# secondmind-labs/trieste

Measured on NVIDIA H100. Metric: acquisition candidate-points/sec (EI on GPR N=4096 fp64), higher is better.
Workload: dtype f64

## Files before the change

trieste_b200/csrc/digit_gemm.cuh:

```cuda
#pragma once
#include "common.cuh"
#include "kernel_fn.cuh"

namespace tb {
namespace oz {

constexpr int KST = 64;
constexpr uint32_t LBO = 128;
constexpr uint32_t SBO = (KST / 16) * 128;
constexpr int ATILE = 128 * KST;

__host__ __device__ inline int64_t a_stage_offset(int I) {
  return (int64_t)I * (I + 1);
}

template <int POS, int SRC>
__device__ __forceinline__ uint32_t put_byte(uint32_t acc, uint32_t w) {
  constexpr uint32_t sel = (POS == 0 ? (4u + SRC) : 0u) | ((POS == 1 ? (4u + SRC) : 1u) << 4) | ((POS == 2 ? (4u + SRC) : 2u) << 8) |
                           ((POS == 3 ? (4u + SRC) : 3u) << 12);
  return __byte_perm(acc, w, sel);
}

}

namespace dg {

using oz::ATILE;
using oz::KST;
using oz::LBO;
using oz::SBO;

constexpr int STAGES = 3;
constexpr int CONSUMER_WARPS = 8;
constexpr int THREADS = CONSUMER_WARPS * 32 + 128;
constexpr int PRODUCER_REGS = 40, CONSUMER_REGS = 232;
enum { EPI_SUMSQ = 0, EPI_STORE = 1 };

template <int S> __host__ __device__ constexpr int chunk_cols() { return S >= 6 ? 32 : 64; }
template <int S> __host__ __device__ constexpr int stage_bytes() { return S * (ATILE + chunk_cols<S>() * KST); }
template <int S> __host__ __device__ constexpr size_t smem_bytes() {
  return (size_t)STAGES * stage_bytes<S>() + 256 + (size_t)CONSUMER_WARPS * chunk_cols<S>() * sizeof(double);
}

__device__ __forceinline__ uint64_t smem_desc(uint32_t saddr) {
  return (uint64_t)((saddr >> 4) & 0x3FFF) | ((uint64_t)((LBO >> 4) & 0x3FFF) << 16) | ((uint64_t)((SBO >> 4) & 0x3FFF) << 32);
}

__device__ __forceinline__ void wgmma_fence() { asm volatile("wgmma.fence.sync.aligned;" ::: "memory"); }
__device__ __forceinline__ void wgmma_commit() { asm volatile("wgmma.commit_group.sync.aligned;" ::: "memory"); }
template <int N>
__device__ __forceinline__ void wgmma_wait() { asm volatile("wgmma.wait_group.sync.aligned %0;" ::"n"(N) : "memory"); }

template <int R>
// ... 28 lines not shown
}
#undef TB_R4

template <int S, int NR>
__device__ __forceinline__ void fence_acc(uint32_t (&acc)[S][NR]) {
#pragma unroll
  for (int l = 0; l < S; ++l)
#pragma unroll
    for (int i = 0; i < NR; ++i) asm volatile("" : "+r"(acc[l][i])::"memory");
}

__device__ __forceinline__ double int_to_double(uint32_t t) {
  return __hiloint2double(0x43300000, (int)(t ^ 0x80000000u)) - 4503601774854144.0;
}

template <int S, int EPI, int NTB>
__global__ void __launch_bounds__(THREADS, 1)
digit_gemm_kernel(const int8_t* __restrict__ AS, const int8_t* __restrict__ BS, const double* __restrict__ rowscale,
                  const double* __restrict__ rowsum, int NB, int nst, int G, int tiles, int64_t McPad, double out_scale,
                  double half_var, int a_planes, int b_planes, int full_rows, double* __restrict__ partial,
                  double* __restrict__ Aplain, int64_t lda) {
  constexpr int CN = chunk_cols<S>(), NCH = NTB / CN, BCH = CN * KST, BTILE = NTB * KST, STAGE = stage_bytes<S>(), NR = CN / 2;
  static_assert(NTB % CN == 0, "a candidate tile is a whole number of column chunks");
  extern __shared__ __align__(1024) unsigned char smem[];
  uint64_t* full = reinterpret_cast<uint64_t*>(smem + (size_t)STAGES * STAGE);
  uint64_t* empty = full + STAGES;
  double (*colbuf)[CN] = reinterpret_cast<double (*)[CN]>(smem + (size_t)STAGES * STAGE + 256);

  const int warp = threadIdx.x >> 5, lane = threadIdx.x & 31;
  const int nitems = tiles * NCH * G;
  if (threadIdx.x == 0) {
    for (int s = 0; s < STAGES; ++s) {
      mbar_init(&full[s], 1);
      mbar_init(&empty[s], CONSUMER_WARPS);
    }
    fence_barrier_init();
  }
  for (int i = threadIdx.x; i < CONSUMER_WARPS * CN; i += blockDim.x) colbuf[i / CN][i % CN] = 0.0;
  __syncthreads();

  if (warp >= CONSUMER_WARPS) {
    setmaxnreg_dec<PRODUCER_REGS>();
    if (warp == CONSUMER_WARPS && lane == 0) {
      int st = 0;
      uint32_t ph = 0;
      for (int item = blockIdx.x; item < nitems; item += gridDim.x) {
        const int g = item % G, tc = item / G, tile = tc / NCH, c = tc % NCH;
        const int8_t* bTile = BS + (int64_t)tile * nst * ((int64_t)b_planes * BTILE) + (int64_t)c * BCH;
        for (int i = 0;; ++i) {
          const int I = serpentine_rowblock(i, g, G);
          if (I >= NB) break;
          const int nk = full_rows ? nst : min(2 * (I + 1), nst);
          const int8_t* aRow = AS + (full_rows ? (int64_t)I * nst : oz::a_stage_offset(I)) * ((int64_t)a_planes * ATILE);
          for (int kc = 0; kc < nk; ++kc) {
            mbar_wait(&empty[st], ph ^ 1);
            unsigned char* dst = smem + (size_t)st * STAGE;
            mbar_expect_tx(&full[st], STAGE);
            bulk_g2s(dst, aRow + (int64_t)kc * ((int64_t)a_planes * ATILE), S * ATILE, &full[st]);
            const int8_t* b = bTile + (int64_t)kc * ((int64_t)b_planes * BTILE);
#pragma unroll
            for (int p = 0; p < S; ++p) bulk_g2s(dst + S * ATILE + p * BCH, b + (int64_t)p * BTILE, BCH, &full[st]);
            if (++st == STAGES) { st = 0; ph ^= 1; }
          }
        }
      }
    }
    return;
  }

  setmaxnreg_inc<CONSUMER_REGS>();
  const int wg = warp >> 2, wq = warp & 3;
  const uint32_t a_lane = (uint32_t)((wg * 8 + wq * 2 + ((lane >> 3) & 1)) * (int)SBO + (lane >> 4) * (int)LBO + (lane & 7) * 16);
  uint32_t acc[S][NR];
  int st = 0;
  uint32_t ph = 0;
  for (int item = blockIdx.x; item < nitems; item += gridDim.x) {
    const int g = item % G, tc = item / G, tile = tc / NCH, c = tc % NCH;
    for (int i = 0;; ++i) {
      const int I = serpentine_rowblock(i, g, G);
      if (I >= NB) break;
      const int nk = full_rows ? nst : min(2 * (I + 1), nst);
#pragma unroll
      for (int l = 0; l < S; ++l)
#pragma unroll
        for (int j = 0; j < NR; ++j) acc[l][j] = 0u;
      fence_acc(acc);
      int held = -1;
      for (int kc = 0; kc < nk; ++kc) {
        mbar_wait(&full[st], ph);
        const uint32_t base = smem_u32(smem + (size_t)st * STAGE);
        const uint64_t b0 = smem_desc(base + (uint32_t)(S * ATILE));
#pragma unroll
        for (int p = 1; p <= S; ++p) {
          uint32_t a[KST / 32][4];
#pragma unroll
          for (int kk = 0; kk < KST / 32; ++kk) ldmatrix_x4(a[kk], base + a_lane + (uint32_t)((p - 1) * ATILE + kk * 2 * (int)LBO));
          wgmma_wait<1>();
          if (p == 2 && held >= 0) {
            __syncwarp();
            if (lane == 0) mbar_arrive(&empty[held]);
          }
          wgmma_fence();
#pragma unroll
          for (int q = 1; q <= S + 1 - p; ++q)
#pragma unroll
            for (int kk = 0; kk < KST / 32; ++kk) wgmma_s8(acc[p + q - 2], a[kk], b0 + (uint64_t)(((q - 1) * BCH + kk * 2 * (int)LBO) >> 4));
          wgmma_commit();
        }
        held = st;
        if (++st == STAGES) { st = 0; ph ^= 1; }
      }
      wgmma_wait<0>();
      fence_acc(acc);
      __syncwarp();
      if (lane == 0) mbar_arrive(&empty[held]);
      const int64_t r0 = (int64_t)I * 128 + wg * 64 + wq * 16 + (lane >> 2), r1 = r0 + 8;
      const double rs0 = rowscale[r0] * out_scale * 0x1p-16, rs1 = rowscale[r1] * out_scale * 0x1p-16;
      const double rc0 = rowsum ? rowsum[r0] * half_var : 0.0, rc1 = rowsum ? rowsum[r1] * half_var : 0.0;
#pragma unroll
      for (int j = 0; j < CN / 8; ++j) {
        double a[4];
#pragma unroll
        for (int e = 0; e < 4; ++e) {
          double v = int_to_double(acc[S - 1][4 * j + e]);
#pragma unroll
          for (int l = S - 2; l >= 0; --l) v = fma(v, 0x1p-8, int_to_double(acc[l][4 * j + e]));
          a[e] = e < 2 ? fma(v, rs0, rc0) : fma(v, rs1, rc1);
        }
        const int col = 8 * j + 2 * (lane & 3);
        if (EPI == EPI_STORE) {
          double* dst = Aplain + ((int64_t)tile * NTB + (int64_t)c * CN + col) * lda;
          dst[r0] = a[0];
          dst[lda + r0] = a[1];
          dst[r1] = a[2];
          dst[lda + r1] = a[3];
        } else {
          double s0 = fma(a[0], a[0], a[2] * a[2]), s1 = fma(a[1], a[1], a[3] * a[3]);
#pragma unroll
          for (int o = 4; o < 32; o <<= 1) {
            s0 += __shfl_xor_sync(0xffffffffu, s0, o);
            s1 += __shfl_xor_sync(0xffffffffu, s1, o);
          }
          if (lane < 4) {
            colbuf[warp][col] += s0;
            colbuf[warp][col + 1] += s1;
          }
        }
      }
    }
    if (EPI == EPI_SUMSQ) {
      asm volatile("bar.sync 1, %0;" ::"n"(CONSUMER_WARPS * 32) : "memory");
      if (threadIdx.x < CN) {
        double s = 0.0;
#pragma unroll
        for (int w = 0; w < CONSUMER_WARPS; ++w) {
          s += colbuf[w][threadIdx.x];
          colbuf[w][threadIdx.x] = 0.0;
        }
        partial[(int64_t)g * McPad + (int64_t)tile * NTB + (int64_t)c * CN + threadIdx.x] = s;
      }
      asm volatile("bar.sync 1, %0;" ::"n"(CONSUMER_WARPS * 32) : "memory");
    }
  }
}

inline int sm_count(int* n) {
  int dev = 0;
  TB_CUDA(cudaGetDevice(&dev));
  TB_CUDA(cudaDeviceGetAttribute(n, cudaDevAttrMultiProcessorCount, dev));
  return 0;
}

template <int S, int EPI, int NTB>
inline int set_smem() {
  TB_CUDA(cudaFuncSetAttribute(digit_gemm_kernel<S, EPI, NTB>, cudaFuncAttributeMaxDynamicSharedMemorySize, (int)smem_bytes<S>()));
  return 0;
}

template <int S, int EPI, int NTB>
inline int launch(cudaStream_t st, const int8_t* AS, const int8_t* BS, const double* rowscale, const double* rowsum, int NB, int nst,
                  int G, int tiles, int64_t McPad, double out_scale, double half_var, int a_planes, int b_planes, int full_rows,
                  double* partial, double* Aplain, int64_t lda) {
  int sms = 0;
  TB_TRY(sm_count(&sms));
  const int64_t items = (int64_t)tiles * (NTB / chunk_cols<S>()) * G;
  const int grid = (int)std::min<int64_t>(sms, items);
  if (grid <= 0) return 0;
  digit_gemm_kernel<S, EPI, NTB><<<grid, THREADS, smem_bytes<S>(), st>>>(AS, BS, rowscale, rowsum, NB, nst, G, tiles, McPad, out_scale,
                                                                         half_var, a_planes, b_planes, full_rows, partial, Aplain, lda);
  TB_LAUNCHED();
  TB_CUDA(cudaGetLastError());
  return 0;
}

}
}
```

trieste_b200/csrc/gp_handle.cuh:

```cuda
#pragma once
#include "common.cuh"
#include "../../include/trieste_b200.h"
#include <cublas_v2.h>
#include <cusolverDn.h>
#include <vector>
#include <algorithm>
#include <cmath>
#include <cstdlib>
#include <type_traits>
#include <utility>

namespace tb {

struct DevBuf {
  void* p = nullptr;
  size_t cap = 0;
  DevBuf() = default;
  DevBuf(const DevBuf&) = delete;
  DevBuf& operator=(const DevBuf&) = delete;
  DevBuf(DevBuf&& o) noexcept : p(o.p), cap(o.cap) {
    o.p = nullptr;
    o.cap = 0;
  }
  DevBuf& operator=(DevBuf&& o) noexcept {
// ... 155 lines not shown
  tb::DevBuf sKs, sPartial, sMean, sVals, sVar, sXc, sBlkBest, sBlkIdx, sRun;
  tb::DevBuf sA, sV, sGrad, sMisc;
  tb::DevBuf dXspare, dyspare, dLspare, dLinvSpare;
  tb::DevBuf dMes;
  int mesS = 0;
  tb::DevBuf dPen;
  int penP = 0, penKind = 0, penD = 0;
  std::vector<double> gibP;
  int gibM = 0, gibMp = 0, gibD = 0;
  double gibW = 0.0;
  uint64_t cache_gen = 0;
  uint64_t gib_gen = tb::STALE;
  tb::DevBuf dGibPs, dGibLinv, dGibWhat;
  tb::DevBuf sGib;
  tb::DevBuf sScrUb, sScrX, sScrIdx, sScrBlk;
  tb::DevBuf dPreRows, dPreCentre;
  uint64_t pre_gen = tb::STALE;
  bool pre_tc = false;
  int pre_nsl = 0, pre_npos_sl = 0;
  double pre_scale = 1.0, pre_x2max = 0.0, pre_rel = 0.0, pre_lin = 0.0, pre_lin_max = 0.0, pre_abs = 0.0;

  bool profile = false;
  double prof_ms = 0.0, prof_flops = 0.0;
  int64_t prof_launches = 0;
  std::vector<std::pair<cudaEvent_t, cudaEvent_t>> prof_events;
  std::vector<double> prof_event_flops;
};
```

trieste_b200/csrc/int8_engines.cu:

```cuda
#include "gp_handle.cuh"
#include "ozaki5.cuh"
#include "int8_engines.h"

namespace tb {

int int8_init() {
  TB_TRY((dg::set_smem<6, dg::EPI_SUMSQ, oz::Geo<6>::NT>()));
  TB_TRY((dg::set_smem<6, dg::EPI_STORE, oz::Geo<6>::NT>()));
  TB_TRY((dg::set_smem<5, dg::EPI_SUMSQ, oz::Geo<5>::NT>()));
  TB_TRY((dg::set_smem<5, dg::EPI_STORE, oz::Geo<5>::NT>()));
  TB_TRY((dg::set_smem<4, dg::EPI_SUMSQ, oz::Geo<4>::NT>()));
  TB_TRY((dg::set_smem<4, dg::EPI_STORE, oz::Geo<4>::NT>()));
  TB_TRY((dg::set_smem<3, dg::EPI_SUMSQ, oz::Geo<3>::NT>()));
  return 0;
}

static int nst_of(const tb_gp* gp) { return (int)((gp->N + oz::KST - 1) / oz::KST); }

static int stored_planes(const tb_gp* gp, bool single_pass) { return single_pass ? gp->digits.linv.planes : oz::S21; }
int int8_tile_width(const tb_gp* gp, bool single_pass) {
  return stored_planes(gp, single_pass) == 5 ? oz::Geo<5>::NT : oz::Geo<6>::NT;
}
size_t int8_tile_bytes(const tb_gp* gp, bool single_pass) {
  return (size_t)nst_of(gp) * stored_planes(gp, single_pass) * int8_tile_width(gp, single_pass) * oz::KST;
}


static int row_stats(tb_gp* gp, DigitOperand& o, const double* A, int full, bool tight) {
// ... 160 lines not shown
  const double* il = gp->dInvLs.as<double>();
  const int N = (int)gp->N, nst = nst_of(gp), D = gp->D;
  const double var = gp->variance, mc0 = gp->mean_const;
  const double inv_b = std::ldexp(1.0, 48 - bscale_exp(var));
  cudaStream_t st = gp->stream;
  with_kind_dp(gp->kernel, gp->DP, [&](auto K, auto P) {
    oz::kstar_digits_kernel<decltype(K)::value, decltype(P)::value><<<tiles, 512, 0, st>>>(Xs, al, Xc_dev, il, N, nst, D, mc, var, inv_b,
                                                                                            mc0, BS, mean);
  });
  TB_LAUNCHED();
  TB_CUDA(cudaGetLastError());
  return 0;
}

template <int S>
static int kstar_single_pass(tb_gp* gp, const double* Xc_dev, int64_t mc, int tiles, int8_t* BS, double* mean, const KSplit* split) {
  const double* Xs = gp->dXs.as<double>();
  const double* al = gp->dAlpha.as<double>();
  const double* il = gp->dInvLs.as<double>();
  const int N = (int)gp->N, nst = nst_of(gp), D = gp->D;
  const double var = gp->variance, mc0 = gp->mean_const;
  const double inv_b = oz::two_pow_8S<S>() * oz::FILL / (0.5 * var);
  const double dig_c = fm::MAGIC + oz5::dig_koff<S>() - centre_int(S);
  const double* X2 = gp->digits.X2.as<double>();
  cudaStream_t st = gp->stream;
  constexpr int TH = oz5::KGEN_WARPS * 32;
  const unsigned ctas = kstar_ctas<S>(tiles);
  const KSplit ks = split ? *split : int8_kstar_split(gp, true, tiles);
  const int ksplit = ks.ksplit, kc_per = ks.kc_per;
  const int64_t mstride = (int64_t)tiles * oz::Geo<S>::NT;
  double* mean_dst = mean;
  if (ksplit > 1) {
    TB_TRY(gp->sMeanPart.reserve(sizeof(double) * (size_t)ksplit * mstride));
    mean_dst = gp->sMeanPart.as<double>();
  }
  with_kind_dp(gp->kernel, gp->DP, [&](auto K, auto P) {
    oz5::kstar_digits_kernel<decltype(K)::value, decltype(P)::value, S><<<dim3(ctas, ksplit), TH, 0, st>>>(
        Xs, X2, al, Xc_dev, il, N, nst, D, mc, var, inv_b, dig_c, mc0, fm::Consts(), tiles, kc_per, BS, mean_dst);
  });
  TB_LAUNCHED();
  if (ksplit > 1) {
    oz5::mean_reduce_kernel<<<(unsigned)((mstride + 255) / 256), 256, 0, st>>>(mean_dst, ksplit, mstride, mc0, mean);
    TB_LAUNCHED();
  }
  TB_CUDA(cudaGetLastError());
  return 0;
}

int int8_kstar(tb_gp* gp, bool single_pass, const double* Xc_dev, int64_t mc, int tiles, int8_t* BS, double* mean,
               const KSplit* split) {
  if (!single_pass) return kstar_21(gp, Xc_dev, mc, tiles, BS, mean);
  return gp->digits.linv.planes == 5 ? kstar_single_pass<5>(gp, Xc_dev, mc, tiles, BS, mean, split)
                                     : kstar_single_pass<4>(gp, Xc_dev, mc, tiles, BS, mean, split);
}


template <int EPI>
static int digit_gemm(tb_gp* gp, const DigitOperand& left, int full_rows, int S, double out_scale, double h, const int8_t* BS,
                      int tiles, int G, int64_t McPad, double* partial, double* out, int64_t lda) {
  auto launch = [&](auto SV) {
    constexpr int s = decltype(SV)::value;
    return dg::launch<s, EPI, oz::Geo<s>::NT>(gp->stream, left.digits.as<int8_t>(), BS, left.scale.as<double>(), left.sum.as<double>(),
                                              gp->NB, nst_of(gp), G, tiles, McPad, out_scale, h, left.planes, left.planes, full_rows,
                                              partial, out, lda);
  };
  switch (S) {
    case 6: return launch(std::integral_constant<int, 6>{});
    case 5: return launch(std::integral_constant<int, 5>{});
    case 4: return launch(std::integral_constant<int, 4>{});
  }
  if constexpr (EPI == dg::EPI_SUMSQ) return launch(std::integral_constant<int, 3>{});
  return fail("digit GEMM: no store kernel computes with " + std::to_string(S) + " digits", ERR_RUNTIME);
}

int int8_variance(tb_gp* gp, bool single_pass, const int8_t* BS, int tiles, int G, int64_t McPad, double* partial) {
  const DigitState& d = gp->digits;
  const double var = gp->variance;
  if (single_pass)
    return digit_gemm<dg::EPI_SUMSQ>(gp, d.linv, 0, d.mode, 0.5 * var / oz::FILL, h_eff(var, d.linv.planes), BS, tiles, G, McPad,
                                     partial, nullptr, 0);
  return digit_gemm<dg::EPI_SUMSQ>(gp, d.linv21, 0, gp->dtype == TB_F32 ? 4 : 6, std::ldexp(1.0, bscale_exp(var)), 0.0, BS, tiles, G,
                                   McPad, partial, nullptr, 0);
}

int int8_store(tb_gp* gp, bool single_pass, bool kinv, const int8_t* BS, int tiles, int G, int64_t McPad, double* out, int64_t lda) {
  const DigitState& d = gp->digits;
  const double var = gp->variance;
  if (single_pass) {
    const DigitOperand& left = kinv ? d.kinv : d.linv;
    return digit_gemm<dg::EPI_STORE>(gp, left, kinv, left.planes, 0.5 * var / oz::FILL, h_eff(var, left.planes), BS, tiles, G, McPad,
                                     nullptr, out, lda);
  }
  return digit_gemm<dg::EPI_STORE>(gp, kinv ? d.kinv21 : d.linv21, kinv, gp->dtype == TB_F32 ? 4 : 6, std::ldexp(1.0, bscale_exp(var)),
                                   0.0, BS, tiles, G, McPad, nullptr, out, lda);
}

}
// ... 1 lines not shown
```

trieste_b200/csrc/int8_engines.h:

```cpp
#pragma once
#include <cuda_runtime.h>
#include <cstddef>
#include <cstdint>
struct tb_gp;
namespace tb {
int int8_init();
int int8_select(tb_gp* gp, bool need_v, bool* single_pass);
int int8_tile_width(const tb_gp* gp, bool single_pass);
size_t int8_tile_bytes(const tb_gp* gp, bool single_pass);
struct KSplit {
  int ksplit = 1, kc_per = 0;
};
KSplit int8_kstar_split(const tb_gp* gp, bool single_pass, int tiles);
int int8_kstar(tb_gp* gp, bool single_pass, const double* Xc_dev, int64_t mc, int tiles, int8_t* BS, double* mean,
               const KSplit* split = nullptr);
int int8_variance(tb_gp* gp, bool single_pass, const int8_t* BS, int tiles, int G, int64_t McPad, double* partial);
int int8_store(tb_gp* gp, bool single_pass, bool kinv, const int8_t* BS, int tiles, int G, int64_t McPad, double* out, int64_t lda);
void int8_info(const tb_gp* gp, int* products, double* estimate);
void int8_pin_full(tb_gp* gp, bool full);
}
```

trieste_b200/csrc/ozaki5.cuh:

```cuda
#pragma once
#include "ozaki.cuh"

namespace tb {
namespace oz5 {

using oz::FILL;
using oz::Geo;
using oz::KST;
using oz::LBO;
using oz::SBO;
using oz::two_pow_8S;

template <int S> __host__ __device__ constexpr double dig_koff() { return S == 5 ? 551911719040.0 : S == 4 ? 2155905152.0 : 8421504.0; }

__global__ void row_norms_kernel(const double* __restrict__ Xs, int64_t rows_have, int DP, int64_t rows, double* __restrict__ X2) {
  const int64_t k = (int64_t)blockIdx.x * blockDim.x + threadIdx.x;
  if (k >= rows) return;
  double s = 0.0;
  if (k < rows_have)
    for (int d = 0; d < DP; ++d) s = fma(Xs[k * DP + d], Xs[k * DP + d], s);
  X2[k] = s;
}

constexpr int KGEN_WARPS = 8;
template <int KIND, int DP, int S>
__global__ void __launch_bounds__(KGEN_WARPS * 32, DP <= 12 ? 4 : 3)
kstar_digits_kernel(const double* __restrict__ Xs, const double* __restrict__ X2, const double* __restrict__ alpha,
                    const double* __restrict__ Xc, const double* __restrict__ inv_ls, int N, int nst, int D, int64_t M, double variance,
                    double inv_bscale_2p, double dig_c, double mean_const, const __grid_constant__ fm::Consts fc, int ntiles,
                    int kc_per, int8_t* __restrict__ BS, double* __restrict__ mean_out) {
  constexpr int NT = Geo<S>::NT, BTILE = NT * KST, TH = KGEN_WARPS * 32, WPT = NT / 8;
  constexpr bool EXPAND = KIND != TB_MATERN12;
  const int lane = threadIdx.x & 31;
  const int64_t wg = (int64_t)blockIdx.x * KGEN_WARPS + (threadIdx.x >> 5);
  const int64_t tile_id = wg / WPT;
  const int w = (int)(wg % WPT);
  const int cl = lane & 7, ch = lane >> 3;
  const int t_local = w * 8 + cl;
  const int64_t t = tile_id * NT + t_local;
  const bool valid = t < M && tile_id < ntiles;
  double xc[DP];
// ... 20 lines not shown
      if (e < CH) asm volatile("cp.async.ca.shared.global [%0], [%1], 16;" ::"r"(smem_u32(&xs_s[buf][2 * e + 2 * blk])), "l"(src + 2 * e) : "memory");
    }
    if (threadIdx.x < KST / 2) {
      const int e = threadIdx.x;
      asm volatile("cp.async.ca.shared.global [%0], [%1], 16;" ::"r"(smem_u32(&al_s[buf][2 * e + 2 * (e / 8)])), "l"(alpha + (int64_t)kc * KST + 2 * e)
                   : "memory");
    } else if (EXPAND && threadIdx.x < KST) {
      const int e = threadIdx.x - KST / 2;
      asm volatile("cp.async.ca.shared.global [%0], [%1], 16;" ::"r"(smem_u32(&x2_s[buf][2 * e + 2 * (e / 8)])), "l"(X2 + (int64_t)kc * KST + 2 * e)
                   : "memory");
    }
    asm volatile("cp.async.commit_group;" ::: "memory");
  };
  const int kc0 = (int)blockIdx.y * kc_per, kc1 = min(nst, kc0 + kc_per);
  stage_load(kc0, 0);
  double macc = 0.0;
  for (int kc = kc0; kc < kc1; ++kc) {
    const int buf = (kc - kc0) & 1;
    if (kc + 1 < kc1) {
      stage_load(kc + 1, buf ^ 1);
      asm volatile("cp.async.wait_group 1;" ::: "memory");
    } else {
      asm volatile("cp.async.wait_group 0;" ::: "memory");
    }
    __syncthreads();
    uint32_t pk[S][4];
#pragma unroll
    for (int p = 0; p < S; ++p) pk[p][0] = pk[p][1] = pk[p][2] = pk[p][3] = 0u;
#pragma unroll
    for (int j = 0; j < 16; ++j) {
      const int kl = ch * 16 + j, kv = kl + 2 * ch;
// ... 7 lines not shown
          dot = fma(xc[d], v.x, dot);
          dot = fma(xc[d + 1], v.y, dot);
        }
        r2 = fma(-2.0, dot, xc2 + x2_s[buf][kv]);
      } else {
        r2 = 0.0;
#pragma unroll
        for (int d = 0; d < DP; d += 2) {
          const double2 v = *reinterpret_cast<const double2*>(xr + d);
          double d0 = xc[d] - v.x, d1 = xc[d + 1] - v.y;
          r2 = fma(d0, d0, r2);
          r2 = fma(d1, d1, r2);
        }
      }
      const double kval = kernel_from_r2_fast<KIND>(r2, variance, exp_tab, fc);
      macc = fma(kval, al_s[buf][kv], macc);
      const double tb = fma(kval, inv_bscale_2p, dig_c);
      const uint32_t wl = (uint32_t)__double2loint(tb) ^ 0x80808080u, wh = (uint32_t)__double2hiint(tb) ^ 0x80u;
      oz::scatter_rt<S>(pk, j, wl, wh);
    }
    if (tile_id < ntiles) {
#pragma unroll
      for (int p = 0; p < S; ++p)
        *reinterpret_cast<uint4*>(tile + (int64_t)kc * (S * BTILE) + p * BTILE) = make_uint4(pk[p][0], pk[p][1], pk[p][2], pk[p][3]);
    }
    __syncthreads();
  }
  macc += __shfl_xor_sync(0xffffffffu, macc, 8);
  macc += __shfl_xor_sync(0xffffffffu, macc, 16);
  if (ch == 0 && tile_id < ntiles)
    mean_out[(int64_t)blockIdx.y * ntiles * NT + tile_id * NT + t_local] = gridDim.y == 1 ? macc + mean_const : macc;
}

__global__ void mean_reduce_kernel(const double* __restrict__ part, int ksplit, int64_t stride, double mean_const,
                                   double* __restrict__ mean_out) {
  const int64_t t = (int64_t)blockIdx.x * blockDim.x + threadIdx.x;
  if (t >= stride) return;
  double s = 0.0;
  for (int i = 0; i < ksplit; ++i) s += part[(int64_t)i * stride + t];
  mean_out[t] = s + mean_const;
}

}
}
```

trieste_b200/csrc/tb_api.cu:

```cuda
#include "gp_handle.cuh"
#include "kernels_extra.cuh"
#include "prescreen.cuh"
#include "batch_ei.cuh"
#include "int8_engines.h"
#include <chrono>
#include "factor.cuh"
#include "lbfgs.cuh"

using namespace tb;
namespace tb {
int kernels_init();
}

namespace tb {

__global__ void scale_inputs_kernel(const double* __restrict__ X, const double* __restrict__ inv_ls,
                                    int64_t N, int D, int DP, int64_t rows, double* __restrict__ Xs) {
  int64_t i = (int64_t)blockIdx.x * blockDim.x + threadIdx.x;
  if (i >= rows * DP) return;
  int64_t k = i / DP;
  int d = (int)(i % DP);
  Xs[i] = (k < N && d < D) ? X[k * D + d] * inv_ls[d] : 0.0;
}

// ... 1065 lines not shown
  *eng = single_pass ? Engine::OZ15 : Engine::OZ21;
  return 0;
}

static int eng_tile_width(const tb_gp* gp, Engine e) { return e == Engine::F64 ? BT : int8_tile_width(gp, e == Engine::OZ15); }
static size_t eng_tile_bytes(const tb_gp* gp, Engine e) {
  return e == Engine::F64 ? (size_t)gp->nkc * PANEL * sizeof(double) : int8_tile_bytes(gp, e == Engine::OZ15);
}

static int eng_groups(const tb_gp* gp, Engine e, int tiles) {
  const int fill = (2 * NUM_SMS + tiles - 1) / tiles;
  if (e == Engine::F64) return tiles >= NUM_SMS ? 1 : std::max(1, std::min(fill, gp->NB));
  return std::max(std::max(1, (gp->NB + 3) / 4), std::min(gp->NB, fill));
}

static int eng_kstar(tb_gp* gp, Engine e, const double* xc, int64_t mc, int tiles, const KSplit* split = nullptr) {
  double* mean = gp->sMean.as<double>();
  if (e == Engine::F64) return launch_kstar(gp, xc, mc, tiles, gp->sKs.as<double>(), mean);
  return int8_kstar(gp, e == Engine::OZ15, xc, mc, tiles, gp->sKs.as<int8_t>(), mean, split);
}

static int eng_variance(tb_gp* gp, Engine e, int tiles, int G, int64_t McPad, bool packed_a) {
  cudaStream_t st = gp->stream;
  double* partial = gp->sPartial.as<double>();
  if (e != Engine::F64) return int8_variance(gp, e == Engine::OZ15, gp->sKs.as<int8_t>(), tiles, G, McPad, partial);
  if (packed_a)
    trigemm_kernel<false, EPI_SUMSQ_PACKED><<<dim3(tiles, G), TG_THREADS, TG_SMEM, st>>>(
        gp->dLinvP.as<double>(), gp->sKs.as<double>(), gp->NB, gp->nkc, G, McPad, partial, gp->sA.as<double>(), nullptr, 0);
  else
    trigemm_kernel<false, EPI_SUMSQ><<<dim3(tiles, G), TG_THREADS, TG_SMEM, st>>>(
        gp->dLinvP.as<double>(), gp->sKs.as<double>(), gp->NB, gp->nkc, G, McPad, partial, nullptr, nullptr, 0);
  TB_LAUNCHED();
  TB_CUDA(cudaGetLastError());
  return 0;
}

static int eng_store_a(tb_gp* gp, Engine e, int tiles, int64_t McPad, double* out) {
  const int64_t lda = (int64_t)gp->NB * BM;
  const int G = eng_groups(gp, e, tiles);
  if (e != Engine::F64) return int8_store(gp, e == Engine::OZ15, false, gp->sKs.as<int8_t>(), tiles, G, McPad, out, lda);
// ... 68 lines not shown
  return 0;
}

struct EvalOut {
  double *vals = nullptr, *mean = nullptr, *var = nullptr, *grad = nullptr;
};

static int eval_chunk(tb_gp* gp, const EvalRequest& rq, Engine e, const double* xc, int64_t n, int64_t c0, int G, const EvalOut& o,
                      const int64_t* idx_map = nullptr, const KSplit* split = nullptr) {
  cudaStream_t st = gp->stream;
  const int nt = eng_tile_width(gp, e);
  const int tiles = (int)((n + nt - 1) / nt);
  const int64_t McPad = (int64_t)tiles * nt;
  const double* partial = gp->sPartial.as<double>();
  const double* mean = gp->sMean.as<double>();
  TB_TRY(eng_kstar(gp, e, xc, n, tiles, split));
  TB_TRY(profiled_gemm(gp, (double)McPad * (double)gp->N * (double)gp->N,
                       [&] { return eng_variance(gp, e, tiles, G, McPad, o.grad != nullptr); }));
  if (o.grad) {
    TB_TRY(launch_partials(gp, st, rq.acq, rq.param, partial, G, McPad, mean, xc, n));
    TB_TRY(eng_store_v(gp, e, tiles, McPad));
    TB_TRY(launch_grad(gp, xc, n, o.grad));
  }
  TB_TRY(launch_tail(gp, st, rq, partial, G, McPad, mean, n, c0, o.vals, o.mean, o.var, xc, o.grad, idx_map));
  return rq.want_argmax ? argmax_fold(gp, n) : 0;
}

static int argmax_screened(tb_gp* gp, const EvalRequest& rq, Engine e, int64_t chunk_cap, int G, bool* done) {
  *done = false;
  cudaStream_t st = gp->stream;
  const int D = gp->D, nt = eng_tile_width(gp, e);
  const int64_t M = rq.M;
  const int64_t cap = std::max<int64_t>(1, M / 4);
// ... 1517 lines not shown
```

Before: 275.9 million.

## Add split-K digit GEMM and wide k-star generation for small candidate batches

When there are too few candidate tiles to fill the SMs (the screened-argmax path with an index map), the int8 digit GEMM splits each row block's K range across CTAs. Partial integer accumulators are combined with atomics into a global buffer and a separate epilogue kernel turns them into variance partial sums. The k-star generation also switches to a wide grid split over K stages, writing kernel values to global memory so that a replay kernel computes the mean. This raises parallelism for small batches at the cost of extra memsets, atomics, global traffic and kernel launches.

```diff
diff --git a/trieste_b200/csrc/digit_gemm.cuh b/trieste_b200/csrc/digit_gemm.cuh
--- a/trieste_b200/csrc/digit_gemm.cuh
+++ b/trieste_b200/csrc/digit_gemm.cuh
@@ -34,9 +34,10 @@
 constexpr int CONSUMER_WARPS = 8;
 constexpr int THREADS = CONSUMER_WARPS * 32 + 128;
 constexpr int PRODUCER_REGS = 40, CONSUMER_REGS = 232;
-enum { EPI_SUMSQ = 0, EPI_STORE = 1 };
-
-template <int S> __host__ __device__ constexpr int chunk_cols() { return S >= 6 ? 32 : 64; }
+enum { EPI_SUMSQ = 0, EPI_STORE = 1, EPI_SPLIT = 2 };
+
+__host__ __device__ constexpr int chunk_cols_of(int S) { return S >= 6 ? 32 : 64; }
+template <int S> __host__ __device__ constexpr int chunk_cols() { return chunk_cols_of(S); }
 template <int S> __host__ __device__ constexpr int stage_bytes() { return S * (ATILE + chunk_cols<S>() * KST); }
 template <int S> __host__ __device__ constexpr size_t smem_bytes() {
   return (size_t)STAGES * stage_bytes<S>() + 256 + (size_t)CONSUMER_WARPS * chunk_cols<S>() * sizeof(double);
@@ -95,12 +96,99 @@
   return __hiloint2double(0x43300000, (int)(t ^ 0x80000000u)) - 4503601774854144.0;
 }
 
+__host__ __device__ inline int rowblock_stages(int I, int nst, int full_rows) { return full_rows ? nst : min(2 * (I + 1), nst); }
+
+__host__ __device__ inline int split_units(int NB, int nst, int full_rows, int kper) {
+  int u = 0;
+  for (int I = 0; I < NB; ++I) u += (rowblock_stages(I, nst, full_rows) + kper - 1) / kper;
+  return u;
+}
+
+template <int EPI>
+__device__ __forceinline__ bool item_range(int g, int i, int G, int NB, int nst, int full_rows, int kper, int& I, int& k0, int& k1) {
+  if constexpr (EPI == EPI_SPLIT) {
+    if (i > 0) return false;
+    for (I = 0; I < NB; ++I) {
+      const int nk = rowblock_stages(I, nst, full_rows), p = (nk + kper - 1) / kper;
+      if (g < p) {
+        k0 = g * kper;
+        k1 = min(nk, k0 + kper);
+        return true;
+      }
+      g -= p;
+    }
+    return false;
+  } else {
+    I = serpentine_rowblock(i, g, G);
+    k0 = 0;
+    k1 = rowblock_stages(I, nst, full_rows);
+    return I < NB;
+  }
+}
+
+template <int S, int EPI, int NTB>
+__device__ __forceinline__ void rowblock_epilogue(const uint32_t (&acc)[S][chunk_cols<S>() / 2], int I, int tile, int c, int warp, int lane,
+                                                  const double* __restrict__ rowscale, const double* __restrict__ rowsum,
+                                                  double out_scale, double half_var, double (*colbuf)[chunk_cols<S>()],
+                                                  double* __restrict__ Aplain, int64_t lda) {
+  constexpr int CN = chunk_cols<S>();
+  const int wg = warp >> 2, wq = warp & 3;
+  const int64_t r0 = (int64_t)I * 128 + wg * 64 + wq * 16 + (lane >> 2), r1 = r0 + 8;
+  const double rs0 = rowscale[r0] * out_scale * 0x1p-16, rs1 = rowscale[r1] * out_scale * 0x1p-16;
+  const double rc0 = rowsum ? rowsum[r0] * half_var : 0.0, rc1 = rowsum ? rowsum[r1] * half_var : 0.0;
+#pragma unroll
+  for (int j = 0; j < CN / 8; ++j) {
+    double a[4];
+#pragma unroll
+    for (int e = 0; e < 4; ++e) {
+      double v = int_to_double(acc[S - 1][4 * j + e]);
+#pragma unroll
+      for (int l = S - 2; l >= 0; --l) v = fma(v, 0x1p-8, int_to_double(acc[l][4 * j + e]));
+      a[e] = e < 2 ? fma(v, rs0, rc0) : fma(v, rs1, rc1);
+    }
+    const int col = 8 * j + 2 * (lane & 3);
+    if constexpr (EPI == EPI_STORE) {
+      double* dst = Aplain + ((int64_t)tile * NTB + (int64_t)c * CN + col) * lda;
+      dst[r0] = a[0];
+      dst[lda + r0] = a[1];
+      dst[r1] = a[2];
+      dst[lda + r1] = a[3];
+    } else {
+      double s0 = fma(a[0], a[0], a[2] * a[2]), s1 = fma(a[1], a[1], a[3] * a[3]);
+#pragma unroll
+      for (int o = 4; o < 32; o <<= 1) {
+        s0 += __shfl_xor_sync(0xffffffffu, s0, o);
+        s1 += __shfl_xor_sync(0xffffffffu, s1, o);
+      }
+      if (lane < 4) {
+        colbuf[warp][col] += s0;
+        colbuf[warp][col + 1] += s1;
+      }
+    }
+  }
+}
+
+template <int CN>
+__device__ __forceinline__ void colbuf_flush(double (*colbuf)[CN], double* __restrict__ dst) {
+  asm volatile("bar.sync 1, %0;" ::"n"(CONSUMER_WARPS * 32) : "memory");
+  if (threadIdx.x < CN) {
+    double s = 0.0;
+#pragma unroll
+    for (int w = 0; w < CONSUMER_WARPS; ++w) {
+      s += colbuf[w][threadIdx.x];
+      colbuf[w][threadIdx.x] = 0.0;
+    }
+    dst[threadIdx.x] = s;
+  }
+  asm volatile("bar.sync 1, %0;" ::"n"(CONSUMER_WARPS * 32) : "memory");
+}
+
 template <int S, int EPI, int NTB>
 __global__ void __launch_bounds__(THREADS, 1)
 digit_gemm_kernel(const int8_t* __restrict__ AS, const int8_t* __restrict__ BS, const double* __restrict__ rowscale,
                   const double* __restrict__ rowsum, int NB, int nst, int G, int tiles, int64_t McPad, double out_scale,
                   double half_var, int a_planes, int b_planes, int full_rows, double* __restrict__ partial,
-                  double* __restrict__ Aplain, int64_t lda) {
+                  double* __restrict__ Aplain, int64_t lda, int kper, int* __restrict__ acc_out) {
   constexpr int CN = chunk_cols<S>(), NCH = NTB / CN, BCH = CN * KST, BTILE = NTB * KST, STAGE = stage_bytes<S>(), NR = CN / 2;
   static_assert(NTB % CN == 0, "a candidate tile is a whole number of column chunks");
   extern __shared__ __align__(1024) unsigned char smem[];
@@ -128,12 +216,10 @@
       for (int item = blockIdx.x; item < nitems; item += gridDim.x) {
         const int g = item % G, tc = item / G, tile = tc / NCH, c = tc % NCH;
         const int8_t* bTile = BS + (int64_t)tile * nst * ((int64_t)b_planes * BTILE) + (int64_t)c * BCH;
-        for (int i = 0;; ++i) {
-          const int I = serpentine_rowblock(i, g, G);
-          if (I >= NB) break;
-          const int nk = full_rows ? nst : min(2 * (I + 1), nst);
+        int I, k0, k1;
+        for (int i = 0; item_range<EPI>(g, i, G, NB, nst, full_rows, kper, I, k0, k1); ++i) {
           const int8_t* aRow = AS + (full_rows ? (int64_t)I * nst : oz::a_stage_offset(I)) * ((int64_t)a_planes * ATILE);
-          for (int kc = 0; kc < nk; ++kc) {
+          for (int kc = k0; kc < k1; ++kc) {
             mbar_wait(&empty[st], ph ^ 1);
             unsigned char* dst = smem + (size_t)st * STAGE;
             mbar_expect_tx(&full[st], STAGE);
@@ -157,17 +243,15 @@
   uint32_t ph = 0;
   for (int item = blockIdx.x; item < nitems; item += gridDim.x) {
     const int g = item % G, tc = item / G, tile = tc / NCH, c = tc % NCH;
-    for (int i = 0;; ++i) {
-      const int I = serpentine_rowblock(i, g, G);
-      if (I >= NB) break;
-      const int nk = full_rows ? nst : min(2 * (I + 1), nst);
+    int I, k0, k1;
+    for (int i = 0; item_range<EPI>(g, i, G, NB, nst, full_rows, kper, I, k0, k1); ++i) {
 #pragma unroll
       for (int l = 0; l < S; ++l)
 #pragma unroll
         for (int j = 0; j < NR; ++j) acc[l][j] = 0u;
       fence_acc(acc);
       int held = -1;
-      for (int kc = 0; kc < nk; ++kc) {
+      for (int kc = k0; kc < k1; ++kc) {
         mbar_wait(&full[st], ph);
         const uint32_t base = smem_u32(smem + (size_t)st * STAGE);
         const uint64_t b0 = smem_desc(base + (uint32_t)(S * ATILE));
@@ -195,54 +279,42 @@
       fence_acc(acc);
       __syncwarp();
       if (lane == 0) mbar_arrive(&empty[held]);
-      const int64_t r0 = (int64_t)I * 128 + wg * 64 + wq * 16 + (lane >> 2), r1 = r0 + 8;
-      const double rs0 = rowscale[r0] * out_scale * 0x1p-16, rs1 = rowscale[r1] * out_scale * 0x1p-16;
-      const double rc0 = rowsum ? rowsum[r0] * half_var : 0.0, rc1 = rowsum ? rowsum[r1] * half_var : 0.0;
-#pragma unroll
-      for (int j = 0; j < CN / 8; ++j) {
-        double a[4];
-#pragma unroll
-        for (int e = 0; e < 4; ++e) {
-          double v = int_to_double(acc[S - 1][4 * j + e]);
-#pragma unroll
-          for (int l = S - 2; l >= 0; --l) v = fma(v, 0x1p-8, int_to_double(acc[l][4 * j + e]));
-          a[e] = e < 2 ? fma(v, rs0, rc0) : fma(v, rs1, rc1);
-        }
-        const int col = 8 * j + 2 * (lane & 3);
-        if (EPI == EPI_STORE) {
-          double* dst = Aplain + ((int64_t)tile * NTB + (int64_t)c * CN + col) * lda;
-          dst[r0] = a[0];
-          dst[lda + r0] = a[1];
-          dst[r1] = a[2];
-          dst[lda + r1] = a[3];
-        } else {
-          double s0 = fma(a[0], a[0], a[2] * a[2]), s1 = fma(a[1], a[1], a[3] * a[3]);
-#pragma unroll
-          for (int o = 4; o < 32; o <<= 1) {
-            s0 += __shfl_xor_sync(0xffffffffu, s0, o);
-            s1 += __shfl_xor_sync(0xffffffffu, s1, o);
-          }
-          if (lane < 4) {
-            colbuf[warp][col] += s0;
-            colbuf[warp][col + 1] += s1;
-          }
-        }
-      }
-    }
-    if (EPI == EPI_SUMSQ) {
-      asm volatile("bar.sync 1, %0;" ::"n"(CONSUMER_WARPS * 32) : "memory");
-      if (threadIdx.x < CN) {
-        double s = 0.0;
-#pragma unroll
-        for (int w = 0; w < CONSUMER_WARPS; ++w) {
-          s += colbuf[w][threadIdx.x];
-          colbuf[w][threadIdx.x] = 0.0;
-        }
-        partial[(int64_t)g * McPad + (int64_t)tile * NTB + (int64_t)c * CN + threadIdx.x] = s;
-      }
-      asm volatile("bar.sync 1, %0;" ::"n"(CONSUMER_WARPS * 32) : "memory");
-    }
-  }
+      if constexpr (EPI == EPI_SPLIT) {
+        int* dst = acc_out + ((int64_t)tc * NB + I) * (S * NR * CONSUMER_WARPS * 32) + threadIdx.x;
+#pragma unroll
+        for (int l = 0; l < S; ++l)
+#pragma unroll
+          for (int j = 0; j < NR; ++j) atomicAdd(dst + (l * NR + j) * (CONSUMER_WARPS * 32), (int)acc[l][j]);
+      } else {
+        rowblock_epilogue<S, EPI, NTB>(acc, I, tile, c, warp, lane, rowscale, rowsum, out_scale, half_var, colbuf, Aplain, lda);
+      }
+    }
+    if constexpr (EPI == EPI_SUMSQ) colbuf_flush<CN>(colbuf, partial + (int64_t)g * McPad + (int64_t)tile * NTB + (int64_t)c * CN);
+  }
+}
+
+template <int S, int NTB>
+__global__ void __launch_bounds__(CONSUMER_WARPS * 32, 1)
+split_epilogue_kernel(const int* __restrict__ acc_in, const double* __restrict__ rowscale, const double* __restrict__ rowsum, int NB,
+                      int G, int64_t McPad, double out_scale, double half_var, double* __restrict__ partial) {
+  constexpr int CN = chunk_cols<S>(), NCH = NTB / CN, NR = CN / 2;
+  __shared__ double colbuf[CONSUMER_WARPS][CN];
+  const int warp = threadIdx.x >> 5, lane = threadIdx.x & 31;
+  const int g = blockIdx.x % G, tc = blockIdx.x / G, tile = tc / NCH, c = tc % NCH;
+  for (int i = threadIdx.x; i < CONSUMER_WARPS * CN; i += blockDim.x) colbuf[i / CN][i % CN] = 0.0;
+  __syncthreads();
+  for (int i = 0;; ++i) {
+    const int I = serpentine_rowblock(i, g, G);
+    if (I >= NB) break;
+    const int* src = acc_in + ((int64_t)tc * NB + I) * (S * NR * CONSUMER_WARPS * 32) + threadIdx.x;
+    uint32_t acc[S][NR];
+#pragma unroll
+    for (int l = 0; l < S; ++l)
+#pragma unroll
+      for (int j = 0; j < NR; ++j) acc[l][j] = (uint32_t)src[(l * NR + j) * (CONSUMER_WARPS * 32)];
+    rowblock_epilogue<S, EPI_SUMSQ, NTB>(acc, I, tile, c, warp, lane, rowscale, rowsum, out_scale, half_var, colbuf, nullptr, 0);
+  }
+  colbuf_flush<CN>(colbuf, partial + (int64_t)g * McPad + (int64_t)tile * NTB + (int64_t)c * CN);
 }
 
 inline int sm_count(int* n) {
@@ -261,18 +333,47 @@
 template <int S, int EPI, int NTB>
 inline int launch(cudaStream_t st, const int8_t* AS, const int8_t* BS, const double* rowscale, const double* rowsum, int NB, int nst,
                   int G, int tiles, int64_t McPad, double out_scale, double half_var, int a_planes, int b_planes, int full_rows,
-                  double* partial, double* Aplain, int64_t lda) {
+                  double* partial, double* Aplain, int64_t lda, int kper = 0, int* acc = nullptr) {
   int sms = 0;
   TB_TRY(sm_count(&sms));
   const int64_t items = (int64_t)tiles * (NTB / chunk_cols<S>()) * G;
   const int grid = (int)std::min<int64_t>(sms, items);
   if (grid <= 0) return 0;
   digit_gemm_kernel<S, EPI, NTB><<<grid, THREADS, smem_bytes<S>(), st>>>(AS, BS, rowscale, rowsum, NB, nst, G, tiles, McPad, out_scale,
-                                                                         half_var, a_planes, b_planes, full_rows, partial, Aplain, lda);
+                                                                         half_var, a_planes, b_planes, full_rows, partial, Aplain, lda,
+                                                                         kper, acc);
   TB_LAUNCHED();
   TB_CUDA(cudaGetLastError());
   return 0;
 }
 
-}
-}
+inline int split_kper(int S, int NTB, int tiles, int G, int NB, int nst, int full_rows) {
+  const int nch = NTB / chunk_cols_of(S);
+  if ((int64_t)tiles * nch * G >= NUM_SMS) return 0;
+  int64_t stages = 0;
+  for (int I = 0; I < NB; ++I) stages += rowblock_stages(I, nst, full_rows);
+  stages *= (int64_t)tiles * nch;
+  int kper = (int)std::min<int64_t>(nst, std::max<int64_t>(8, (stages + NUM_SMS - 1) / NUM_SMS));
+  while (kper < nst && (int64_t)tiles * nch * split_units(NB, nst, full_rows, kper) > NUM_SMS) ++kper;
+  return kper;
+}
+template <int S> inline size_t split_acc_bytes(int tiles, int NTB, int NB) {
+  return (size_t)tiles * (NTB / chunk_cols<S>()) * NB * S * (chunk_cols<S>() / 2) * (CONSUMER_WARPS * 32) * sizeof(int);
+}
+
+template <int S, int NTB>
+inline int launch_split(cudaStream_t st, const int8_t* AS, const int8_t* BS, const double* rowscale, const double* rowsum, int NB,
+                        int nst, int G, int tiles, int64_t McPad, double out_scale, double half_var, int a_planes, int b_planes,
+                        int full_rows, int kper, int* acc, double* partial) {
+  TB_CUDA(cudaMemsetAsync(acc, 0, split_acc_bytes<S>(tiles, NTB, NB), st));
+  TB_TRY((launch<S, EPI_SPLIT, NTB>(st, AS, BS, rowscale, rowsum, NB, nst, split_units(NB, nst, full_rows, kper), tiles, McPad,
+                                    out_scale, half_var, a_planes, b_planes, full_rows, nullptr, nullptr, 0, kper, acc)));
+  split_epilogue_kernel<S, NTB><<<tiles * (NTB / chunk_cols<S>()) * G, CONSUMER_WARPS * 32, 0, st>>>(acc, rowscale, rowsum, NB, G, McPad,
+                                                                                                   out_scale, half_var, partial);
+  TB_LAUNCHED();
+  TB_CUDA(cudaGetLastError());
+  return 0;
+}
+
+}
+}
diff --git a/trieste_b200/csrc/gp_handle.cuh b/trieste_b200/csrc/gp_handle.cuh
--- a/trieste_b200/csrc/gp_handle.cuh
+++ b/trieste_b200/csrc/gp_handle.cuh
@@ -193,6 +193,7 @@
   tb::DevBuf dGibPs, dGibLinv, dGibWhat;
   tb::DevBuf sGib;
   tb::DevBuf sScrUb, sScrX, sScrIdx, sScrBlk;
+  tb::DevBuf sKval, sSplitAcc;
   tb::DevBuf dPreRows, dPreCentre;
   uint64_t pre_gen = tb::STALE;
   bool pre_tc = false;
diff --git a/trieste_b200/csrc/int8_engines.cu b/trieste_b200/csrc/int8_engines.cu
--- a/trieste_b200/csrc/int8_engines.cu
+++ b/trieste_b200/csrc/int8_engines.cu
@@ -12,6 +12,10 @@
   TB_TRY((dg::set_smem<4, dg::EPI_SUMSQ, oz::Geo<4>::NT>()));
   TB_TRY((dg::set_smem<4, dg::EPI_STORE, oz::Geo<4>::NT>()));
   TB_TRY((dg::set_smem<3, dg::EPI_SUMSQ, oz::Geo<3>::NT>()));
+  TB_TRY((dg::set_smem<6, dg::EPI_SPLIT, oz::Geo<6>::NT>()));
+  TB_TRY((dg::set_smem<5, dg::EPI_SPLIT, oz::Geo<5>::NT>()));
+  TB_TRY((dg::set_smem<4, dg::EPI_SPLIT, oz::Geo<4>::NT>()));
+  TB_TRY((dg::set_smem<3, dg::EPI_SPLIT, oz::Geo<3>::NT>()));
   return 0;
 }
 
@@ -202,7 +206,8 @@
 }
 
 template <int S>
-static int kstar_single_pass(tb_gp* gp, const double* Xc_dev, int64_t mc, int tiles, int8_t* BS, double* mean, const KSplit* split) {
+static int kstar_single_pass(tb_gp* gp, const double* Xc_dev, int64_t mc, int tiles, int8_t* BS, double* mean, const KSplit* split,
+                             bool wide) {
   const double* Xs = gp->dXs.as<double>();
   const double* al = gp->dAlpha.as<double>();
   const double* il = gp->dInvLs.as<double>();
@@ -217,6 +222,22 @@
   const KSplit ks = split ? *split : int8_kstar_split(gp, true, tiles);
   const int ksplit = ks.ksplit, kc_per = ks.kc_per;
   const int64_t mstride = (int64_t)tiles * oz::Geo<S>::NT;
+  if (wide) {
+    const int wsplit = (int)std::min<int64_t>(nst, (4 * NUM_SMS + ctas - 1) / ctas);
+    const int wkc = (nst + wsplit - 1) / wsplit;
+    TB_TRY(gp->sKval.reserve(sizeof(double) * (size_t)nst * oz::KST * mstride));
+    double* kval = gp->sKval.as<double>();
+    with_kind_dp(gp->kernel, gp->DP, [&](auto K, auto P) {
+      oz5::kstar_digits_kernel<decltype(K)::value, decltype(P)::value, S, true><<<dim3(ctas, (nst + wkc - 1) / wkc), TH, 0, st>>>(
+          Xs, X2, al, Xc_dev, il, N, nst, D, mc, var, inv_b, dig_c, mc0, fm::Consts(), tiles, wkc, BS, kval);
+    });
+    TB_LAUNCHED();
+    oz5::mean_replay_kernel<<<(unsigned)(mstride * 4 / oz5::REPLAY_THREADS), oz5::REPLAY_THREADS, 0, st>>>(kval, al, nst, ksplit, kc_per,
+                                                                                                        mstride, mc0, mean);
+    TB_LAUNCHED();
+    TB_CUDA(cudaGetLastError());
+    return 0;
+  }
   double* mean_dst = mean;
   if (ksplit > 1) {
     TB_TRY(gp->sMeanPart.reserve(sizeof(double) * (size_t)ksplit * mstride));
@@ -236,21 +257,34 @@
 }
 
 int int8_kstar(tb_gp* gp, bool single_pass, const double* Xc_dev, int64_t mc, int tiles, int8_t* BS, double* mean,
-               const KSplit* split) {
+               const KSplit* split, bool wide) {
   if (!single_pass) return kstar_21(gp, Xc_dev, mc, tiles, BS, mean);
-  return gp->digits.linv.planes == 5 ? kstar_single_pass<5>(gp, Xc_dev, mc, tiles, BS, mean, split)
-                                     : kstar_single_pass<4>(gp, Xc_dev, mc, tiles, BS, mean, split);
+  return gp->digits.linv.planes == 5 ? kstar_single_pass<5>(gp, Xc_dev, mc, tiles, BS, mean, split, wide)
+                                     : kstar_single_pass<4>(gp, Xc_dev, mc, tiles, BS, mean, split, wide);
+}
+
+static int variance_digits(const tb_gp* gp, bool single_pass) { return single_pass ? gp->digits.mode : gp->dtype == TB_F32 ? 4 : 6; }
+
+int int8_split_kper(const tb_gp* gp, bool single_pass, int tiles, int G) {
+  return dg::split_kper(variance_digits(gp, single_pass), int8_tile_width(gp, single_pass), tiles, G, gp->NB, nst_of(gp), 0);
 }
 
 
 template <int EPI>
 static int digit_gemm(tb_gp* gp, const DigitOperand& left, int full_rows, int S, double out_scale, double h, const int8_t* BS,
-                      int tiles, int G, int64_t McPad, double* partial, double* out, int64_t lda) {
+                      int tiles, int G, int64_t McPad, double* partial, double* out, int64_t lda, int kper = 0) {
   auto launch = [&](auto SV) {
-    constexpr int s = decltype(SV)::value;
-    return dg::launch<s, EPI, oz::Geo<s>::NT>(gp->stream, left.digits.as<int8_t>(), BS, left.scale.as<double>(), left.sum.as<double>(),
-                                              gp->NB, nst_of(gp), G, tiles, McPad, out_scale, h, left.planes, left.planes, full_rows,
-                                              partial, out, lda);
+    constexpr int s = decltype(SV)::value, NT = oz::Geo<s>::NT;
+    if constexpr (EPI == dg::EPI_SUMSQ) {
+      if (kper > 0) {
+        TB_TRY(gp->sSplitAcc.reserve(dg::split_acc_bytes<s>(tiles, NT, gp->NB)));
+        return dg::launch_split<s, NT>(gp->stream, left.digits.as<int8_t>(), BS, left.scale.as<double>(), left.sum.as<double>(), gp->NB,
+                                       nst_of(gp), G, tiles, McPad, out_scale, h, left.planes, left.planes, full_rows, kper,
+                                       gp->sSplitAcc.as<int>(), partial);
+      }
+    }
+    return dg::launch<s, EPI, NT>(gp->stream, left.digits.as<int8_t>(), BS, left.scale.as<double>(), left.sum.as<double>(), gp->NB,
+                                  nst_of(gp), G, tiles, McPad, out_scale, h, left.planes, left.planes, full_rows, partial, out, lda);
   };
   switch (S) {
     case 6: return launch(std::integral_constant<int, 6>{});
@@ -261,14 +295,15 @@
   return fail("digit GEMM: no store kernel computes with " + std::to_string(S) + " digits", ERR_RUNTIME);
 }
 
-int int8_variance(tb_gp* gp, bool single_pass, const int8_t* BS, int tiles, int G, int64_t McPad, double* partial) {
+int int8_variance(tb_gp* gp, bool single_pass, const int8_t* BS, int tiles, int G, int64_t McPad, double* partial, int kper) {
   const DigitState& d = gp->digits;
   const double var = gp->variance;
+  const int S = variance_digits(gp, single_pass);
   if (single_pass)
-    return digit_gemm<dg::EPI_SUMSQ>(gp, d.linv, 0, d.mode, 0.5 * var / oz::FILL, h_eff(var, d.linv.planes), BS, tiles, G, McPad,
-                                     partial, nullptr, 0);
-  return digit_gemm<dg::EPI_SUMSQ>(gp, d.linv21, 0, gp->dtype == TB_F32 ? 4 : 6, std::ldexp(1.0, bscale_exp(var)), 0.0, BS, tiles, G,
-                                   McPad, partial, nullptr, 0);
+    return digit_gemm<dg::EPI_SUMSQ>(gp, d.linv, 0, S, 0.5 * var / oz::FILL, h_eff(var, d.linv.planes), BS, tiles, G, McPad, partial,
+                                     nullptr, 0, kper);
+  return digit_gemm<dg::EPI_SUMSQ>(gp, d.linv21, 0, S, std::ldexp(1.0, bscale_exp(var)), 0.0, BS, tiles, G, McPad, partial, nullptr, 0,
+                                   kper);
 }
 
 int int8_store(tb_gp* gp, bool single_pass, bool kinv, const int8_t* BS, int tiles, int G, int64_t McPad, double* out, int64_t lda) {
diff --git a/trieste_b200/csrc/int8_engines.h b/trieste_b200/csrc/int8_engines.h
--- a/trieste_b200/csrc/int8_engines.h
+++ b/trieste_b200/csrc/int8_engines.h
@@ -13,8 +13,9 @@
 };
 KSplit int8_kstar_split(const tb_gp* gp, bool single_pass, int tiles);
 int int8_kstar(tb_gp* gp, bool single_pass, const double* Xc_dev, int64_t mc, int tiles, int8_t* BS, double* mean,
-               const KSplit* split = nullptr);
-int int8_variance(tb_gp* gp, bool single_pass, const int8_t* BS, int tiles, int G, int64_t McPad, double* partial);
+               const KSplit* split = nullptr, bool wide = false);
+int int8_variance(tb_gp* gp, bool single_pass, const int8_t* BS, int tiles, int G, int64_t McPad, double* partial, int kper = 0);
+int int8_split_kper(const tb_gp* gp, bool single_pass, int tiles, int G);
 int int8_store(tb_gp* gp, bool single_pass, bool kinv, const int8_t* BS, int tiles, int G, int64_t McPad, double* out, int64_t lda);
 void int8_info(const tb_gp* gp, int* products, double* estimate);
 void int8_pin_full(tb_gp* gp, bool full);
diff --git a/trieste_b200/csrc/ozaki5.cuh b/trieste_b200/csrc/ozaki5.cuh
--- a/trieste_b200/csrc/ozaki5.cuh
+++ b/trieste_b200/csrc/ozaki5.cuh
@@ -23,8 +23,8 @@
 }
 
 constexpr int KGEN_WARPS = 8;
-template <int KIND, int DP, int S>
-__global__ void __launch_bounds__(KGEN_WARPS * 32, DP <= 12 ? 4 : 3)
+template <int KIND, int DP, int S, bool KVAL = false>
+__global__ void __launch_bounds__(KGEN_WARPS * 32, KVAL ? (DP <= 12 ? 2 : 1) : DP <= 12 ? 4 : 3)
 kstar_digits_kernel(const double* __restrict__ Xs, const double* __restrict__ X2, const double* __restrict__ alpha,
                     const double* __restrict__ Xc, const double* __restrict__ inv_ls, int N, int nst, int D, int64_t M, double variance,
                     double inv_bscale_2p, double dig_c, double mean_const, const __grid_constant__ fm::Consts fc, int ntiles,
@@ -75,7 +75,7 @@
   };
   const int kc0 = (int)blockIdx.y * kc_per, kc1 = min(nst, kc0 + kc_per);
   stage_load(kc0, 0);
-  double macc = 0.0;
+  double macc = 0.0, kprev = 0.0;
   for (int kc = kc0; kc < kc1; ++kc) {
     const int buf = (kc - kc0) & 1;
     if (kc + 1 < kc1) {
@@ -113,7 +113,16 @@
         }
       }
       const double kval = kernel_from_r2_fast<KIND>(r2, variance, exp_tab, fc);
-      macc = fma(kval, al_s[buf][kv], macc);
+      if constexpr (KVAL) {
+        if (!(j & 1)) {
+          kprev = kval;
+        } else if (tile_id < ntiles) {
+          *reinterpret_cast<double2*>(mean_out + (tile_id * NT + t_local) * (int64_t)nst * KST + (int64_t)kc * KST + kl - 1) =
+              make_double2(kprev, kval);
+        }
+      } else {
+        macc = fma(kval, al_s[buf][kv], macc);
+      }
       const double tb = fma(kval, inv_bscale_2p, dig_c);
       const uint32_t wl = (uint32_t)__double2loint(tb) ^ 0x80808080u, wh = (uint32_t)__double2hiint(tb) ^ 0x80u;
       oz::scatter_rt<S>(pk, j, wl, wh);
@@ -125,10 +134,12 @@
     }
     __syncthreads();
   }
-  macc += __shfl_xor_sync(0xffffffffu, macc, 8);
-  macc += __shfl_xor_sync(0xffffffffu, macc, 16);
-  if (ch == 0 && tile_id < ntiles)
-    mean_out[(int64_t)blockIdx.y * ntiles * NT + tile_id * NT + t_local] = gridDim.y == 1 ? macc + mean_const : macc;
+  if constexpr (!KVAL) {
+    macc += __shfl_xor_sync(0xffffffffu, macc, 8);
+    macc += __shfl_xor_sync(0xffffffffu, macc, 16);
+    if (ch == 0 && tile_id < ntiles)
+      mean_out[(int64_t)blockIdx.y * ntiles * NT + tile_id * NT + t_local] = gridDim.y == 1 ? macc + mean_const : macc;
+  }
 }
 
 __global__ void mean_reduce_kernel(const double* __restrict__ part, int ksplit, int64_t stride, double mean_const,
@@ -140,5 +151,44 @@
   mean_out[t] = s + mean_const;
 }
 
+constexpr int REPLAY_THREADS = 64;
+__global__ void __launch_bounds__(REPLAY_THREADS)
+mean_replay_kernel(const double* __restrict__ kval, const double* __restrict__ alpha, int nst, int ksplit, int kc_per, int64_t stride,
+                   double mean_const, double* __restrict__ mean_out) {
+  const int lane = threadIdx.x & 31, cl = lane & 7, ch = lane >> 3;
+  const int64_t t = (((int64_t)blockIdx.x * blockDim.x + threadIdx.x) >> 5) * 8 + cl;
+  if (t - cl >= stride) return;
+  const double* kt = kval + t * (int64_t)nst * KST + ch * 16;
+  double s = 0.0, macc = 0.0;
+  const double* at = alpha + ch * 16;
+  double2 kv[8], av[8];
+  auto load = [&](int kc) {
+#pragma unroll
+    for (int j = 0; j < 8; ++j) {
+      kv[j] = *reinterpret_cast<const double2*>(kt + kc * KST + 2 * j);
+      av[j] = *reinterpret_cast<const double2*>(at + kc * KST + 2 * j);
+    }
+  };
+  load(0);
+  for (int sp = 0; sp < ksplit; ++sp) {
+    const int kc0 = sp * kc_per, kc1 = min(nst, kc0 + kc_per);
+    macc = 0.0;
+    for (int kc = kc0; kc < kc1; ++kc) {
+      const double2 k2[8] = {kv[0], kv[1], kv[2], kv[3], kv[4], kv[5], kv[6], kv[7]};
+      const double2 a2[8] = {av[0], av[1], av[2], av[3], av[4], av[5], av[6], av[7]};
+      if (kc + 1 < nst) load(kc + 1);
+#pragma unroll
+      for (int j = 0; j < 8; ++j) {
+        macc = fma(k2[j].x, a2[j].x, macc);
+        macc = fma(k2[j].y, a2[j].y, macc);
+      }
+    }
+    macc += __shfl_xor_sync(0xffffffffu, macc, 8);
+    macc += __shfl_xor_sync(0xffffffffu, macc, 16);
+    s += macc;
+  }
+  if (ch == 0) mean_out[t] = ksplit == 1 ? macc + mean_const : s + mean_const;
+}
+
 }
 }
diff --git a/trieste_b200/csrc/tb_api.cu b/trieste_b200/csrc/tb_api.cu
--- a/trieste_b200/csrc/tb_api.cu
+++ b/trieste_b200/csrc/tb_api.cu
@@ -1103,16 +1103,16 @@
   return std::max(std::max(1, (gp->NB + 3) / 4), std::min(gp->NB, fill));
 }
 
-static int eng_kstar(tb_gp* gp, Engine e, const double* xc, int64_t mc, int tiles, const KSplit* split = nullptr) {
+static int eng_kstar(tb_gp* gp, Engine e, const double* xc, int64_t mc, int tiles, const KSplit* split = nullptr, bool wide = false) {
   double* mean = gp->sMean.as<double>();
   if (e == Engine::F64) return launch_kstar(gp, xc, mc, tiles, gp->sKs.as<double>(), mean);
-  return int8_kstar(gp, e == Engine::OZ15, xc, mc, tiles, gp->sKs.as<int8_t>(), mean, split);
-}
-
-static int eng_variance(tb_gp* gp, Engine e, int tiles, int G, int64_t McPad, bool packed_a) {
+  return int8_kstar(gp, e == Engine::OZ15, xc, mc, tiles, gp->sKs.as<int8_t>(), mean, split, wide);
+}
+
+static int eng_variance(tb_gp* gp, Engine e, int tiles, int G, int64_t McPad, bool packed_a, int kper = 0) {
   cudaStream_t st = gp->stream;
   double* partial = gp->sPartial.as<double>();
-  if (e != Engine::F64) return int8_variance(gp, e == Engine::OZ15, gp->sKs.as<int8_t>(), tiles, G, McPad, partial);
+  if (e != Engine::F64) return int8_variance(gp, e == Engine::OZ15, gp->sKs.as<int8_t>(), tiles, G, McPad, partial, kper);
   if (packed_a)
     trigemm_kernel<false, EPI_SUMSQ_PACKED><<<dim3(tiles, G), TG_THREADS, TG_SMEM, st>>>(
         gp->dLinvP.as<double>(), gp->sKs.as<double>(), gp->NB, gp->nkc, G, McPad, partial, gp->sA.as<double>(), nullptr, 0);
@@ -1211,9 +1211,10 @@
   const int64_t McPad = (int64_t)tiles * nt;
   const double* partial = gp->sPartial.as<double>();
   const double* mean = gp->sMean.as<double>();
-  TB_TRY(eng_kstar(gp, e, xc, n, tiles, split));
+  const int kper = idx_map && e != Engine::F64 ? int8_split_kper(gp, e == Engine::OZ15, tiles, G) : 0;
+  TB_TRY(eng_kstar(gp, e, xc, n, tiles, split, kper > 0));
   TB_TRY(profiled_gemm(gp, (double)McPad * (double)gp->N * (double)gp->N,
-                       [&] { return eng_variance(gp, e, tiles, G, McPad, o.grad != nullptr); }));
+                       [&] { return eng_variance(gp, e, tiles, G, McPad, o.grad != nullptr, kper); }));
   if (o.grad) {
     TB_TRY(launch_partials(gp, st, rq.acq, rq.param, partial, G, McPad, mean, xc, n));
     TB_TRY(eng_store_v(gp, e, tiles, McPad));
```

Measured after the change: 299.2 million, median of 6. +8.5%, better.
